# luisdiaz1997/GPzoo

Measured on AMD Instinct MI355X. Metric: ELBO evals/sec (L=32-latent evaluations, all GPUs) at M=2048 inducing, N=200000, L=32 latents/GPU x 1 GPU(s), higher is better.
Workload: dtype f32; 1 GPU; BASELINE configs[2]: Slide-seq-shaped synthetic, N=200000 spots, M=2048, L=32 latents/GPU x 1 GPU(s), matern32, f32; latents_total=32, whitened=True, chunk=0, factor_dtype=f64

## Files before the change

### gpzoo_amd/csrc/kgrad.hip

```cpp
#include "common.h"

namespace gpz {

struct KgradArgs {
  const void* Kbar; int64_t ld, stride;
  const void* Z; const void* X;
  const int64_t* gZ; const int64_t* gX;
  const void* sigma; const void* ell; const void* ga; const void* gr2;
  double gpow, scalar_scale;
  int64_t M, ncols, Mp;
  int d, G;
  double* acc;
};

__device__ __forceinline__ float kg_exp(float x) { return __builtin_amdgcn_exp2f(x * 1.44269504088896341f); }
__device__ __forceinline__ double kg_exp(double x) { return exp(x); }
__device__ __forceinline__ float kg_sqrt(float x) { return sqrtf(x); }
__device__ __forceinline__ double kg_sqrt(double x) { return sqrt(x); }
__device__ __forceinline__ float kg_rsqrt(float x) { return rsqrtf(x); }
__device__ __forceinline__ double kg_rsqrt(double x) { return 1.0 / sqrt(x); }
__device__ __forceinline__ float kg_pow(float x, float y) { return __builtin_amdgcn_exp2f(y * __builtin_amdgcn_logf(x)); }
__device__ __forceinline__ double kg_pow(double x, double y) { return pow(x, y); }

template <typename T, int KIND>
__global__ __launch_bounds__(256) void kgrad_kernel(KgradArgs a) {
  const int l = blockIdx.y, wave = threadIdx.x >> 6, lane = threadIdx.x & 63;
  const int64_t m = (int64_t)blockIdx.x * 4 + wave;
  if (m >= a.M) return;
  const T* kb = static_cast<const T*>(a.Kbar) + (int64_t)l * a.stride + m * a.ld;
  const T* Zp = static_cast<const T*>(a.Z);
  const T* Xp = static_cast<const T*>(a.X);
  const int d = a.d;
  const T sig = static_cast<const T*>(a.sigma)[l];
  const T ell = static_cast<const T*>(a.ell)[l];
  const T s2 = sig * sig, il2 = (T)1 / (ell * ell);
  T z[4] = {0, 0, 0, 0};
  for (int k = 0; k < d; ++k) z[k] = Zp[m * d + k];
  const int gz = (KIND == 2) ? ((uint64_t)a.gZ[m] < (uint64_t)a.G ? (int)a.gZ[m] : 0) : 0;
  const T aeff = (KIND == 2) ? static_cast<const T*>(a.ga)[l] : (T)0;
  const T gpow = (T)a.gpow;
  double dz[4] = {0, 0, 0, 0}, dsig = 0, dell = 0, da = 0;
  constexpr int UN = 4;
  for (int64_t c0 = lane; c0 < a.ncols; c0 += 64 * UN) {
    T g[UN], x[UN][4];
    int gx[UN];
#pragma unroll
    for (int u = 0; u < UN; ++u) {
      const int64_t c = c0 + 64 * u;
      const bool in = c < a.ncols;
      g[u] = in ? kb[c] : (T)0;
#pragma unroll
      for (int k = 0; k < 4; ++k) x[u][k] = (in && k < d) ? Xp[c * d + k] : (T)0;
      gx[u] = (KIND == 2 && in) ? ((uint64_t)a.gX[c] < (uint64_t)a.G ? (int)a.gX[c] : 0) : 0;
    }
    T pz[4] = {0, 0, 0, 0}, psig = 0, pell = 0, pa = 0;
#pragma unroll
    for (int u = 0; u < UN; ++u) {
      T diff[4], d2 = 0;
#pragma unroll
      for (int k = 0; k < 4; ++k) { diff[k] = (k < d) ? z[k] - x[u][k] : (T)0; d2 = fma(diff[k], diff[k], d2); }
      T cz;
      if (KIND == 0) {
        const T kv = s2 * kg_exp((T)-0.5 * d2 * il2);
        psig += g[u] * (T)2 * kv / sig;
        pell += g[u] * kv * d2 * il2 / ell;
        cz = -kv * il2;
      } else if (KIND == 1) {
        const T v = (T)1.7320508075688772935 * kg_sqrt(d2) / ell, e = kg_exp(-v);
        psig += g[u] * (T)2 * sig * ((T)1 + v) * e;
        pell += g[u] * s2 * v * v * e / ell;
        cz = -s2 * (T)3 * il2 * e;
      } else if (KIND == 4) {
        const T rr = kg_sqrt(d2), kv = s2 * kg_exp(-rr / ell);
        psig += g[u] * (T)2 * kv / sig;
        pell += g[u] * kv * rr * il2;
        cz = d2 > (T)0 ? -(kv / ell) * kg_rsqrt(d2) : (T)0;
      } else if (KIND == 5) {
        const T v = (T)2.2360679774997896964 * kg_sqrt(d2) / ell, e = kg_exp(-v), q3 = v * v / (T)3;
        psig += g[u] * (T)2 * sig * ((T)1 + v + q3) * e;
        pell += g[u] * s2 * q3 * ((T)1 + v) * e / ell;
        cz = -s2 * (T)5 / (T)3 * il2 * ((T)1 + v) * e;
      } else {
        const T r2 = static_cast<const T*>(a.gr2)[gz * a.G + gx[u]];
        const T den = aeff * r2 + (T)1;
        const T kv = s2 * kg_exp((T)-0.5 * d2 * il2 / den) * kg_pow(den, -gpow);
        psig += g[u] * (T)2 * kv / sig;
        pell += g[u] * kv * d2 * il2 / (ell * den);
        pa += g[u] * kv * ((T)0.5 * d2 * il2 / (den * den) - gpow / den) * r2;
        cz = -kv * il2 / den;
      }
      const T gc = g[u] * cz;
#pragma unroll
      for (int k = 0; k < 4; ++k) pz[k] = fma(gc, diff[k], pz[k]);
    }
    dsig += (double)psig; dell += (double)pell; da += (double)pa;
#pragma unroll
    for (int k = 0; k < 4; ++k) dz[k] += (double)pz[k];
  }
  double v[7] = {dz[0], dz[1], dz[2], dz[3], dsig * a.scalar_scale, dell * a.scalar_scale, da * a.scalar_scale};
#pragma unroll
  for (int i = 0; i < 7; ++i)
    for (int o = 32; o > 0; o >>= 1) v[i] += __shfl_down(v[i], o);
  if (lane == 0) {
    double* dst = a.acc + ((int64_t)l * a.Mp + m) * 8;
#pragma unroll
    for (int i = 0; i < 7; ++i) dst[i] += v[i];
  }
}

int kgrad_launch(int dtype, int kind, const KgradArgs& a, int L, hipStream_t s) {
  GPZ_REQUIRE((kind >= 0 && kind <= 2) || kind == GPZ_KERNEL_MATERN12 || kind == GPZ_KERNEL_MATERN52,
              "kgrad: unknown kernel kind %d", kind);
  dim3 grid((unsigned)((a.M + 3) / 4), (unsigned)L), block(256);
#define GPZ_KG(T, K) hipLaunchKernelGGL((kgrad_kernel<T, K>), grid, block, 0, s, a)
#define GPZ_KG_KINDS(T) \
  switch (kind) { case 0: GPZ_KG(T, 0); break; case 1: GPZ_KG(T, 1); break; case 4: GPZ_KG(T, 4); break; \
                  case 5: GPZ_KG(T, 5); break; default: GPZ_KG(T, 2); break; }
  if (dtype == GPZ_F32) GPZ_KG_KINDS(float) else GPZ_KG_KINDS(double)
#undef GPZ_KG_KINDS
#undef GPZ_KG
  GPZ_LAUNCH_OK();
  return 0;
}

}

namespace gpz {
__global__ __launch_bounds__(256) void kgrad_public_finish_kernel(const double* __restrict__ acc, int L, int64_t M, int d,
                                                                  double* __restrict__ grad_A,
                                                                  double* __restrict__ grad_theta) {
  __shared__ double sh[4];
  if (blockIdx.y == 0) {
    const int64_t m = (int64_t)blockIdx.x * 256 + threadIdx.x;
    if (m < M && grad_A)
      for (int k = 0; k < 4; ++k) {
        double t = 0.0;
        if (k < d)
          for (int l = 0; l < L; ++l) t += acc[((int64_t)l * M + m) * 8 + k];
        grad_A[m * 4 + k] = t;
      }
  } else if ((int)blockIdx.x < L && grad_theta) {
    const int l = blockIdx.x;
    for (int q = 0; q < 3; ++q) {
      double v = 0.0;
      for (int64_t m = threadIdx.x; m < M; m += 256) v += acc[((int64_t)l * M + m) * 8 + 4 + q];
      for (int o = 32; o > 0; o >>= 1) v += __shfl_down(v, o);
      __syncthreads();
      if ((threadIdx.x & 63) == 0) sh[threadIdx.x >> 6] = v;
      __syncthreads();
      if (threadIdx.x == 0) grad_theta[l * 4 + q] = sh[0] + sh[1] + sh[2] + sh[3];
    }
    if (threadIdx.x == 0) grad_theta[l * 4 + 3] = 0.0;
  }
}
}

extern "C" size_t gpz_kgrad_workspace_bytes(int64_t nA, int32_t n_latent) {
  if (nA < 1 || n_latent < 1) return 0;
  gpz::Carver c(nullptr);
  c.take<double>((int64_t)n_latent * nA * 8);
  return c.used();
}

extern "C" int gpz_kgrad(const gpz_kernel_desc* k, const void* A, int64_t nA, const void* B, int64_t nB, int32_t d,
                         const int64_t* gA, const int64_t* gB, const void* Kbar, int64_t ldk, int64_t stride_k,
                         double* grad_theta, double* grad_A, void* ws, size_t ws_bytes, void* stream) {
  using namespace gpz;
  GPZ_REQUIRE(k && A && B && Kbar && ws, "gpz_kgrad: null pointer");
  GPZ_REQUIRE(nA >= 1 && nB >= 1 && ldk >= nB && d >= 1 && d <= 4, "gpz_kgrad: bad extents nA=%lld nB=%lld ldk=%lld d=%d",
              (long long)nA, (long long)nB, (long long)ldk, d);
  GPZ_REQUIRE((k->kind >= 0 && k->kind <= 2) || k->kind == GPZ_KERNEL_MATERN12 || k->kind == GPZ_KERNEL_MATERN52,
              "gpz_kgrad: kernel kind %d has no parameters to differentiate", k->kind);
  GPZ_REQUIRE(k->n_latent >= 1 && (k->dtype == GPZ_F32 || k->dtype == GPZ_F64), "gpz_kgrad: bad kernel description");
  if (k->kind == GPZ_KERNEL_MGGP_RBF)
    GPZ_REQUIRE(gA && gB && k->group_a && k->group_r2 && k->n_groups >= 1, "gpz_kgrad: MGGP kernel needs groups, group_a, group_r2");
  GPZ_REQUIRE(ws_bytes >= gpz_kgrad_workspace_bytes(nA, k->n_latent), "gpz_kgrad: workspace too small");
  hipStream_t s = static_cast<hipStream_t>(stream);
  const int L = k->n_latent;
  Carver c(ws);
  double* acc = c.take<double>((int64_t)L * nA * 8);
  GPZ_HIP_OK(hipMemsetAsync(acc, 0, sizeof(double) * L * nA * 8, s));
  KgradArgs a;
  a.Kbar = Kbar; a.ld = ldk; a.stride = stride_k; a.Z = A; a.X = B; a.gZ = gA; a.gX = gB;
  a.sigma = k->sigma; a.ell = k->lengthscale; a.ga = k->group_a; a.gr2 = k->group_r2;
  a.gpow = k->group_pow; a.scalar_scale = 1.0; a.M = nA; a.ncols = nB; a.Mp = nA; a.d = d; a.G = k->n_groups; a.acc = acc;
  if (int rc = kgrad_launch(k->dtype, k->kind, a, L, s)) return rc;
  const unsigned fx = (unsigned)((nA + 255) / 256 > L ? (nA + 255) / 256 : L);
  hipLaunchKernelGGL(kgrad_public_finish_kernel, dim3(fx, 2), dim3(256), 0, s, acc, L, nA, d, grad_A, grad_theta);
  GPZ_LAUNCH_OK();
  return 0;
}
```

Baseline: 2.639 ELBO evals/s.

## Restructure kgrad kernel with multi-row tiling, vector loads, and factored constants

```diff
diff --git a/gpzoo_amd/csrc/kgrad.hip b/gpzoo_amd/csrc/kgrad.hip
--- a/gpzoo_amd/csrc/kgrad.hip
+++ b/gpzoo_amd/csrc/kgrad.hip
@@ -13,111 +13,203 @@
   double* acc;
 };
 
-__device__ __forceinline__ float kg_exp(float x) { return __builtin_amdgcn_exp2f(x * 1.44269504088896341f); }
-__device__ __forceinline__ double kg_exp(double x) { return exp(x); }
-__device__ __forceinline__ float kg_sqrt(float x) { return sqrtf(x); }
+template <typename T> struct KgExp;
+template <> struct KgExp<float> {
+  static constexpr float L2E = 1.44269504088896341f;
+  static __device__ __forceinline__ float f(float x) { return __builtin_amdgcn_exp2f(x); }
+};
+template <> struct KgExp<double> {
+  static constexpr double L2E = 1.0;
+  static __device__ __forceinline__ double f(double x) { return exp(x); }
+};
+__device__ __forceinline__ float kg_sqrt(float x) { return __builtin_amdgcn_sqrtf(x); }
 __device__ __forceinline__ double kg_sqrt(double x) { return sqrt(x); }
-__device__ __forceinline__ float kg_rsqrt(float x) { return rsqrtf(x); }
+__device__ __forceinline__ float kg_rsqrt(float x) { return __builtin_amdgcn_rsqf(x); }
 __device__ __forceinline__ double kg_rsqrt(double x) { return 1.0 / sqrt(x); }
 __device__ __forceinline__ float kg_pow(float x, float y) { return __builtin_amdgcn_exp2f(y * __builtin_amdgcn_logf(x)); }
 __device__ __forceinline__ double kg_pow(double x, double y) { return pow(x, y); }
 
-template <typename T, int KIND>
+template <typename T> struct alignas(16) KgVec4 { T v[4]; };
+
+template <bool VEC, typename T>
+__device__ __forceinline__ void kg_load4(const T* __restrict__ p, int64_t c, int64_t n, T (&out)[4]) {
+  if (VEC && c + 4 <= n) {
+    const KgVec4<T> t = *reinterpret_cast<const KgVec4<T>*>(p + c);
+#pragma unroll
+    for (int j = 0; j < 4; ++j) out[j] = t.v[j];
+  } else {
+#pragma unroll
+    for (int j = 0; j < 4; ++j) out[j] = c + j < n ? p[c + j] : (T)0;
+  }
+}
+
+constexpr int KG_ROWS = 4, KG_FOLD = 8, KG_MIN_WGS = 2048;
+
+template <typename T, int KIND, int D, bool VEC, int R>
 __global__ __launch_bounds__(256) void kgrad_kernel(KgradArgs a) {
+  constexpr int NS = D + 2 + (KIND == 2 ? 1 : 0);
   const int l = blockIdx.y, wave = threadIdx.x >> 6, lane = threadIdx.x & 63;
-  const int64_t m = (int64_t)blockIdx.x * 4 + wave;
-  if (m >= a.M) return;
-  const T* kb = static_cast<const T*>(a.Kbar) + (int64_t)l * a.stride + m * a.ld;
+  const int64_t m0 = ((int64_t)blockIdx.x * 4 + wave) * R;
+  if (m0 >= a.M) return;
+  const T* kb = static_cast<const T*>(a.Kbar) + (int64_t)l * a.stride;
   const T* Zp = static_cast<const T*>(a.Z);
   const T* Xp = static_cast<const T*>(a.X);
-  const int d = a.d;
   const T sig = static_cast<const T*>(a.sigma)[l];
   const T ell = static_cast<const T*>(a.ell)[l];
-  const T s2 = sig * sig, il2 = (T)1 / (ell * ell);
-  T z[4] = {0, 0, 0, 0};
-  for (int k = 0; k < d; ++k) z[k] = Zp[m * d + k];
-  const int gz = (KIND == 2) ? ((uint64_t)a.gZ[m] < (uint64_t)a.G ? (int)a.gZ[m] : 0) : 0;
+  const T s2 = sig * sig, il = (T)1 / ell, il2 = il * il;
   const T aeff = (KIND == 2) ? static_cast<const T*>(a.ga)[l] : (T)0;
   const T gpow = (T)a.gpow;
-  double dz[4] = {0, 0, 0, 0}, dsig = 0, dell = 0, da = 0;
-  constexpr int UN = 4;
-  for (int64_t c0 = lane; c0 < a.ncols; c0 += 64 * UN) {
-    T g[UN], x[UN][4];
-    int gx[UN];
-#pragma unroll
-    for (int u = 0; u < UN; ++u) {
-      const int64_t c = c0 + 64 * u;
-      const bool in = c < a.ncols;
-      g[u] = in ? kb[c] : (T)0;
-#pragma unroll
-      for (int k = 0; k < 4; ++k) x[u][k] = (in && k < d) ? Xp[c * d + k] : (T)0;
-      gx[u] = (KIND == 2 && in) ? ((uint64_t)a.gX[c] < (uint64_t)a.G ? (int)a.gX[c] : 0) : 0;
-    }
-    T pz[4] = {0, 0, 0, 0}, psig = 0, pell = 0, pa = 0;
-#pragma unroll
-    for (int u = 0; u < UN; ++u) {
-      T diff[4], d2 = 0;
-#pragma unroll
-      for (int k = 0; k < 4; ++k) { diff[k] = (k < d) ? z[k] - x[u][k] : (T)0; d2 = fma(diff[k], diff[k], d2); }
-      T cz;
-      if (KIND == 0) {
-        const T kv = s2 * kg_exp((T)-0.5 * d2 * il2);
-        psig += g[u] * (T)2 * kv / sig;
-        pell += g[u] * kv * d2 * il2 / ell;
-        cz = -kv * il2;
-      } else if (KIND == 1) {
-        const T v = (T)1.7320508075688772935 * kg_sqrt(d2) / ell, e = kg_exp(-v);
-        psig += g[u] * (T)2 * sig * ((T)1 + v) * e;
-        pell += g[u] * s2 * v * v * e / ell;
-        cz = -s2 * (T)3 * il2 * e;
-      } else if (KIND == 4) {
-        const T rr = kg_sqrt(d2), kv = s2 * kg_exp(-rr / ell);
-        psig += g[u] * (T)2 * kv / sig;
-        pell += g[u] * kv * rr * il2;
-        cz = d2 > (T)0 ? -(kv / ell) * kg_rsqrt(d2) : (T)0;
-      } else if (KIND == 5) {
-        const T v = (T)2.2360679774997896964 * kg_sqrt(d2) / ell, e = kg_exp(-v), q3 = v * v / (T)3;
-        psig += g[u] * (T)2 * sig * ((T)1 + v + q3) * e;
-        pell += g[u] * s2 * q3 * ((T)1 + v) * e / ell;
-        cz = -s2 * (T)5 / (T)3 * il2 * ((T)1 + v) * e;
-      } else {
-        const T r2 = static_cast<const T*>(a.gr2)[gz * a.G + gx[u]];
-        const T den = aeff * r2 + (T)1;
-        const T kv = s2 * kg_exp((T)-0.5 * d2 * il2 / den) * kg_pow(den, -gpow);
-        psig += g[u] * (T)2 * kv / sig;
-        pell += g[u] * kv * d2 * il2 / (ell * den);
-        pa += g[u] * kv * ((T)0.5 * d2 * il2 / (den * den) - gpow / den) * r2;
-        cz = -kv * il2 / den;
+  const T ce = KgExp<T>::L2E * (KIND == 0 || KIND == 2 ? (T)-0.5 * il2
+                                : KIND == 1 ? (T)-1.7320508075688772935 * il
+                                : KIND == 4 ? -il : (T)-2.2360679774997896964 * il);
+  const T cv = KIND == 1 ? (T)1.7320508075688772935 * il : (T)2.2360679774997896964 * il;
+  T z[R][D];
+  const T* row[R];
+  int gz[R];
+#pragma unroll
+  for (int i = 0; i < R; ++i) {
+    const int64_t m = m0 + i < a.M ? m0 + i : a.M - 1;
+    row[i] = kb + m * a.ld;
+#pragma unroll
+    for (int k = 0; k < D; ++k) z[i][k] = Zp[m * D + k];
+    gz[i] = (KIND == 2) ? ((uint64_t)a.gZ[m] < (uint64_t)a.G ? (int)a.gZ[m] : 0) : 0;
+  }
+  double tot[R][NS];
+  T part[R][NS];
+#pragma unroll
+  for (int i = 0; i < R; ++i)
+#pragma unroll
+    for (int q = 0; q < NS; ++q) { tot[i][q] = 0.0; part[i][q] = (T)0; }
+  int fold = 0;
+  for (int64_t c = (int64_t)lane * 4; c < a.ncols; c += 256) {
+    T x[D][4];
+    {
+      T xr[D * 4 > 4 ? D * 4 : 4];
+#pragma unroll
+      for (int k = 0; k < D; ++k) {
+        T t[4];
+        kg_load4<VEC>(Xp, c * D + 4 * k, a.ncols * D, t);
+#pragma unroll
+        for (int j = 0; j < 4; ++j) xr[4 * k + j] = t[j];
       }
-      const T gc = g[u] * cz;
-#pragma unroll
-      for (int k = 0; k < 4; ++k) pz[k] = fma(gc, diff[k], pz[k]);
-    }
-    dsig += (double)psig; dell += (double)pell; da += (double)pa;
-#pragma unroll
-    for (int k = 0; k < 4; ++k) dz[k] += (double)pz[k];
-  }
-  double v[7] = {dz[0], dz[1], dz[2], dz[3], dsig * a.scalar_scale, dell * a.scalar_scale, da * a.scalar_scale};
-#pragma unroll
-  for (int i = 0; i < 7; ++i)
-    for (int o = 32; o > 0; o >>= 1) v[i] += __shfl_down(v[i], o);
-  if (lane == 0) {
-    double* dst = a.acc + ((int64_t)l * a.Mp + m) * 8;
-#pragma unroll
-    for (int i = 0; i < 7; ++i) dst[i] += v[i];
+#pragma unroll
+      for (int j = 0; j < 4; ++j)
+#pragma unroll
+        for (int k = 0; k < D; ++k) x[k][j] = xr[j * D + k];
+    }
+    int gx[4] = {0, 0, 0, 0};
+    if (KIND == 2) {
+#pragma unroll
+      for (int j = 0; j < 4; ++j)
+        if (c + j < a.ncols) gx[j] = (uint64_t)a.gX[c + j] < (uint64_t)a.G ? (int)a.gX[c + j] : 0;
+    }
+    T g[R][4];
+#pragma unroll
+    for (int i = 0; i < R; ++i) {
+      kg_load4<VEC>(row[i], c, a.ncols, g[i]);
+    }
+#pragma unroll
+    for (int i = 0; i < R; ++i) {
+#pragma unroll
+      for (int j = 0; j < 4; ++j) {
+        T diff[D], d2 = 0;
+#pragma unroll
+        for (int k = 0; k < D; ++k) { diff[k] = z[i][k] - x[k][j]; d2 = fma(diff[k], diff[k], d2); }
+        T gz_;
+        if (KIND == 0) {
+          const T ge = g[i][j] * KgExp<T>::f(ce * d2);
+          part[i][D] += ge;
+          part[i][D + 1] = fma(ge, d2, part[i][D + 1]);
+          gz_ = ge;
+        } else if (KIND == 1) {
+          const T rr = kg_sqrt(d2), ge = g[i][j] * KgExp<T>::f(ce * rr), gev = ge * (cv * rr);
+          part[i][D] += ge + gev;
+          part[i][D + 1] = fma(gev, cv * rr, part[i][D + 1]);
+          gz_ = ge;
+        } else if (KIND == 4) {
+          const T rr = kg_sqrt(d2), ge = g[i][j] * KgExp<T>::f(ce * rr);
+          part[i][D] += ge;
+          part[i][D + 1] = fma(ge, rr, part[i][D + 1]);
+          gz_ = d2 > (T)0 ? ge * kg_rsqrt(d2) : (T)0;
+        } else if (KIND == 5) {
+          const T rr = kg_sqrt(d2), v = cv * rr, ge = g[i][j] * KgExp<T>::f(ce * rr), q3 = v * v * (T)(1.0 / 3.0);
+          const T ge1 = fma(ge, v, ge);
+          part[i][D] += fma(ge, q3, ge1);
+          part[i][D + 1] = fma(ge1, q3, part[i][D + 1]);
+          gz_ = ge1;
+        } else {
+          const T r2 = static_cast<const T*>(a.gr2)[gz[i] * a.G + gx[j]];
+          const T den = aeff * r2 + (T)1, iden = (T)1 / den, q = d2 * iden;
+          const T ge = g[i][j] * KgExp<T>::f(ce * q) * kg_pow(den, -gpow);
+          part[i][D] += ge;
+          part[i][D + 1] = fma(ge, q, part[i][D + 1]);
+          part[i][D + 2] = fma(ge * r2, ((T)0.5 * il2 * q - gpow) * iden, part[i][D + 2]);
+          gz_ = ge * iden;
+        }
+#pragma unroll
+        for (int k = 0; k < D; ++k) part[i][k] = fma(gz_, diff[k], part[i][k]);
+      }
+    }
+    if (++fold == KG_FOLD) {
+      fold = 0;
+#pragma unroll
+      for (int i = 0; i < R; ++i)
+#pragma unroll
+        for (int q = 0; q < NS; ++q) { tot[i][q] += (double)part[i][q]; part[i][q] = (T)0; }
+    }
+  }
+  const double fs = 2.0 * (double)sig * a.scalar_scale;
+  double fz, fl;
+  if (KIND == 0) { fz = -(double)(s2 * il2); fl = (double)(s2 * il2 * il); }
+  else if (KIND == 1) { fz = -(double)(s2 * (T)3 * il2); fl = (double)(s2 * il); }
+  else if (KIND == 4) { fz = -(double)(s2 * il); fl = (double)(s2 * il2); }
+  else if (KIND == 5) { fz = -(double)(s2 * (T)5 / (T)3 * il2); fl = (double)(s2 * il); }
+  else { fz = -(double)(s2 * il2); fl = (double)(s2 * il2 * il); }
+  fl *= a.scalar_scale;
+  const double fa = (double)s2 * a.scalar_scale;
+#pragma unroll
+  for (int i = 0; i < R; ++i) {
+    double v[NS];
+#pragma unroll
+    for (int q = 0; q < NS; ++q) {
+      v[q] = tot[i][q] + (double)part[i][q];
+      for (int o = 32; o > 0; o >>= 1) v[q] += __shfl_down(v[q], o);
+    }
+    if (lane == 0 && m0 + i < a.M) {
+      double* dst = a.acc + ((int64_t)l * a.Mp + m0 + i) * 8;
+#pragma unroll
+      for (int k = 0; k < D; ++k) dst[k] += fz * v[k];
+      dst[4] += fs * v[D];
+      dst[5] += fl * v[D + 1];
+      if (KIND == 2) dst[6] += fa * v[NS - 1];
+    }
   }
 }
 
 int kgrad_launch(int dtype, int kind, const KgradArgs& a, int L, hipStream_t s) {
   GPZ_REQUIRE((kind >= 0 && kind <= 2) || kind == GPZ_KERNEL_MATERN12 || kind == GPZ_KERNEL_MATERN52,
               "kgrad: unknown kernel kind %d", kind);
-  dim3 grid((unsigned)((a.M + 3) / 4), (unsigned)L), block(256);
-#define GPZ_KG(T, K) hipLaunchKernelGGL((kgrad_kernel<T, K>), grid, block, 0, s, a)
+  GPZ_REQUIRE(a.d >= 1 && a.d <= 4, "kgrad: %d input dimensions", a.d);
+  const size_t esz = dtype == GPZ_F32 ? 4 : 8;
+  const bool vec = (a.ld * esz) % 16 == 0 && (a.stride * esz) % 16 == 0 &&
+                   reinterpret_cast<uintptr_t>(a.Kbar) % 16 == 0 && reinterpret_cast<uintptr_t>(a.X) % 16 == 0;
+  const bool many = (a.M + 4 * KG_ROWS - 1) / (4 * KG_ROWS) * L >= KG_MIN_WGS;
+  const int64_t rows_wg = many ? 4 * KG_ROWS : 4;
+  dim3 grid((unsigned)((a.M + rows_wg - 1) / rows_wg), (unsigned)L), block(256);
+#define GPZ_KG(T, K, D) \
+  do { if (vec && many) hipLaunchKernelGGL((kgrad_kernel<T, K, D, true, KG_ROWS>), grid, block, 0, s, a); \
+       else if (vec) hipLaunchKernelGGL((kgrad_kernel<T, K, D, true, 1>), grid, block, 0, s, a); \
+       else if (many) hipLaunchKernelGGL((kgrad_kernel<T, K, D, false, KG_ROWS>), grid, block, 0, s, a); \
+       else hipLaunchKernelGGL((kgrad_kernel<T, K, D, false, 1>), grid, block, 0, s, a); } while (0)
+#define GPZ_KG_D(T, K) \
+  switch (a.d) { case 1: GPZ_KG(T, K, 1); break; case 2: GPZ_KG(T, K, 2); break; case 3: GPZ_KG(T, K, 3); break; \
+                 default: GPZ_KG(T, K, 4); break; }
 #define GPZ_KG_KINDS(T) \
-  switch (kind) { case 0: GPZ_KG(T, 0); break; case 1: GPZ_KG(T, 1); break; case 4: GPZ_KG(T, 4); break; \
-                  case 5: GPZ_KG(T, 5); break; default: GPZ_KG(T, 2); break; }
+  switch (kind) { case 0: GPZ_KG_D(T, 0); break; case 1: GPZ_KG_D(T, 1); break; case 4: GPZ_KG_D(T, 4); break; \
+                  case 5: GPZ_KG_D(T, 5); break; default: GPZ_KG_D(T, 2); break; }
   if (dtype == GPZ_F32) GPZ_KG_KINDS(float) else GPZ_KG_KINDS(double)
 #undef GPZ_KG_KINDS
+#undef GPZ_KG_D
 #undef GPZ_KG
   GPZ_LAUNCH_OK();
   return 0;
```

Result: no change. 2.638 ELBO evals/s, median of 2 (-0.0%).
